# centreborelli/sat-bundleadjust

Hardware: AMD Instinct MI355X
Metric: LM iters/sec at 200 cams x 1M pts x 10M obs (affine, R+T) (higher is better)
Workload: dtype f64; 1 GPU; C4: 200 cams x 1000000 pts x 9998866 obs, affine, correction R+T, 1 fixed camera, seed 1; obs_per_rank0=9998866

## Files before the change

sat-bundleadjust_amd/csrc/satba_capi.hip:

```cpp
#include <hip/hip_runtime.h>

#include <algorithm>
#include <atomic>
#include <chrono>
#include <cmath>
#include <cstdarg>
#include <cstdio>
#include <cstdlib>
#include <cstring>
#include <new>
#include <string>
#include <thread>
#include <vector>

#include "../../include/satba.h"
#include "satba_chol.h"
#include "satba_kernels.h"
#include "satba_layout.h"
#include "satba_lm.h"
#include "satba_lmdev.h"
#include "satba_outliers.h"
#include "satba_triangulate.h"
#include "satba_tracks.h"
#include "satba_ftracks.h"
// ... 399 lines not shown
        while (p->prof_ev.size() < p->prof_used + 2) {
            hipEvent_t e;
            HIP_TRY(hipEventCreate(&e));
            p->prof_ev.push_back(e);
        }
        HIP_TRY(hipEventRecord(p->prof_ev[p->prof_used], p->stream));
    }
    SATBA_DISPATCH(p, TRY((launch_lin<MODEL, NP, CL, RL>(p, a))));
    if (prof) {
        HIP_TRY(hipEventRecord(p->prof_ev[p->prof_used + 1], p->stream));
        p->prof_used += 2;
    }
    return 0;
}

static int launch_cam_sums(satba_problem* p, const int* gate, double* U, double* gc) {
    ObsArgs a = obs_args(p, false, gate);
    CamMajor cm = cam_major(p);
    SATBA_DISPATCH(p, hipLaunchKernelGGL((k_cam_sums<MODEL, NP>), dim3(p->M, p->cm_chunks), dim3(LINC_THREADS), 0, p->stream, a, cm, p->d_f, p->d_part3));
    HIP_TRY(hipGetLastError());
    const int total = p->M * cam_acc_len(p->NP);
    hipLaunchKernelGGL(k_cam_sums_finish, dim3((total + 255) / 256), dim3(256), 0, p->stream, p->M, p->NP, p->cm_chunks, p->d_part3, U, gc, gate);
    HIP_TRY(hipGetLastError());
    return 0;
}

static SchurArgs schur_args(const satba_problem* p) {
    SchurArgs s;
    s.PV = reinterpret_cast<const double2*>(p->d_PV);
    s.pair_ofs = p->L.pair_ofs; s.pair_pts = p->L.pair_pts; s.pair_pi = p->L.pair_pi; s.pair_pj = p->L.pair_pj;
    s.pair_ij = p->L.pair_ij; s.pair_part = p->d_pair_part; s.n_chunks = p->L.C; s.items = p->d_items; s.desc = p->d_item_desc;
    if (wmode(p) && p->L.wl_ready) {
        s.PV = p->d_W; s.wmode = 1; s.zero_fix = p->L.zero_fix; s.n_dg = p->L.n_dg;
        s.pair_rec = p->L.pair_rec; s.pair_kk = p->L.pair_kk; s.cm_rec = p->L.cm_rec; s.cm_sc = p->L.cm_sc; s.dg_part = p->d_part3;
        s.items = p->d_items_w; s.desc = p->d_item_desc_w;
    }
    return s;
}

template <int MODEL, int NP>
static int launch_schur(satba_problem* p, const FrontCtx& f, const ObsArgs& a, double* S, double* rhs) {
    CamMajor cm = cam_major(p);
    SchurArgs s = schur_args(p);
    const long long n_pairs = p->L.n_pairs;
    const bool pairs_run = n_pairs > 0 && p->L.E > 0;
    const bool dg_in_pairs = s.wmode && MODEL != RPC && pairs_run;
    int dchunks = (a.sc && MODEL != RPC) ? p->cm_chunks_w : p->cm_chunks;
    static const bool one_launch_env = !(getenv("SATBA_SCHUR_ONE_LAUNCH") && atoi(getenv("SATBA_SCHUR_ONE_LAUNCH")) == 0);
    const bool both = one_launch_env && !f.arrive_epoch && !dg_in_pairs && pairs_run;
    if (dg_in_pairs) dchunks = p->L.n_dg;
    else {
        if (s.wmode) cm.pt = p->L.cm_rec;
        s.diag_xcd = (dchunks % 8 == 0 && !getenv("SATBA_NO_DIAG_XCD")) ? 1 : 0;
        if (!both) hipLaunchKernelGGL((k_schur_diag<MODEL, NP>), dim3(p->M, dchunks), dim3(LINC_THREADS), 0, p->stream, a, cm, s, p->d_part3);
    }
    const int total = p->M * cam_acc_len(NP);
    const int nb_diag = (int)((std::max<long long>(8ll * total, p->hdr) + 255) / 256);
    auto finish = [&](int red_chunks, bool direct) {
        const long long outs = red_chunks > 1 ? n_pairs * NP * NP : 0;
        const bool scale = f.scale_in_finish && !direct && 1 + CH_MAX_STEPS <= nb_diag * 256;
        hipLaunchKernelGGL(k_schur_finish, dim3((unsigned)(nb_diag + (outs + 255) / 256)), dim3(256), 0, p->stream, p->M, NP, p->n_c, dchunks, p->d_part3,
                           f.lam, f.lam_dev, p->lead, p->d_gc, p->d_scale_inv, S, rhs, p->d_xb, (int)p->hdr, nb_diag, red_chunks,
                           p->L.pair_ij, p->d_pair_part, a.gate, scale ? p->d_dch : (double*)nullptr, scale ? p->d_fail : (int*)nullptr,
                           scale ? 1 + CH_MAX_STEPS : 0);
        p->s_scaled = scale;
    };
    if (f.arrive_epoch) {
        if (dg_in_pairs) {
            const int keep = dchunks;
            dchunks = 0;
            finish(1, true);
            dchunks = keep;
            s.dg_cnt = p->d_dg_cnt; s.dg_lam = f.lam; s.dg_lam_dev = f.lam_dev; s.dg_lead = p->lead; s.dg_gc = p->d_gc;
            s.dg_scale_inv = p->d_scale_inv; s.dg_rhs = rhs;
        } else finish(1, true);
        s.arrive = p->d_arrive; s.arrive_epoch = f.arrive_epoch; s.pair_cnt = p->d_pair_cnt; s.fail = p->d_fail;
    }
    int red_chunks = 1;
    if (n_pairs > 0 && p->L.E > 0) {
        const bool merged = a.unit && p->d_item_desc_merged;
        if (merged) { s.desc = p->d_item_desc_merged; s.items = p->d_items_merged; s.n_chunks = 1; }
        const dim3 igrid((unsigned)(merged ? p->n_item_blocks_merged : (s.wmode ? p->n_item_blocks_w : p->n_item_blocks)));
        if (both) {
            const int n_diag = p->M * dchunks, n_diag_pad = (n_diag + 7) & ~7;
            const dim3 bgrid(igrid.x + (unsigned)n_diag_pad);
            if (a.unit) hipLaunchKernelGGL((k_schur_both<MODEL, NP, true>), bgrid, dim3(256), 0, p->stream, a, cm, s, p->d_part3, S, n_diag, n_diag_pad, p->M, dchunks);
            else hipLaunchKernelGGL((k_schur_both<MODEL, NP, false>), bgrid, dim3(256), 0, p->stream, a, cm, s, p->d_part3, S, n_diag, n_diag_pad, p->M, dchunks);
        }
        else if (a.unit) hipLaunchKernelGGL((k_schur_pairs<MODEL, NP, true>), igrid, dim3(256), 0, p->stream, a, s, S);
        else hipLaunchKernelGGL((k_schur_pairs<MODEL, NP, false>), igrid, dim3(256), 0, p->stream, a, s, S);
        HIP_TRY(hipGetLastError());
        if (p->L.C > 1 && !merged) red_chunks = p->L.C;
        if (f.arrive_epoch && (a.unit ? red_chunks > 1 : false)) return fail(SATBA_E_STATE, "factorisation beside a unit-weight pair kernel with chunk partials");
    }
    if (!f.arrive_epoch) finish(red_chunks, n_pairs > 0 && p->L.E > 0 && red_chunks == 1);
    HIP_TRY(hipGetLastError());
    return 0;
}

static int launch_schur_kernel(satba_problem* p, const int* gate, const FrontCtx& f) {
    ObsArgs a = obs_args(p, false, gate);
    double* S = p->payload();
    double* rhs = S + (size_t)p->n_c * p->n_c;
    SATBA_DISPATCH(p, TRY((launch_schur<MODEL, NP>(p, f, a, S, rhs))));
    return 0;
}

// ... 1407 lines not shown
```

sat-bundleadjust_amd/csrc/satba_schur.h:

```cpp
#pragma once
#include "satba_kernels.h"

namespace satba {

constexpr int PV_STRIDE = 16;
__device__ inline double schur_lambda(const double* __restrict__ hdr, double Delta, double lam_floor, double* __restrict__ keep, bool write) {
    const double gh_sq = hdr[SATBA_HDR_GH_SQ], jg_sq = hdr[SATBA_HDR_JG_SQ], xs_sq = hdr[SATBA_HDR_XS_SQ];
    if (!(Delta > 0.0)) {
        Delta = sqrt(xs_sq);
        if (Delta == 0.0) Delta = 1.0;
    }
    const double a = 0.5 * jg_sq, b = -gh_sq, ub = Delta / sqrt(gh_sq);
    double best = fmin(0.0, a * ub * ub + b * ub);
    if (a != 0.0) {
        const double ext = -0.5 * b / a;
        if (0.0 < ext && ext < ub) best = fmin(best, a * ext * ext + b * ext);
    }
    double lam = -best / (Delta * Delta);
    if (!(lam >= lam_floor)) lam = lam_floor;
    if (write) {
        keep[SATBA_KEEP_GINF] = fmax(keep[SATBA_KEEP_GINF], hdr[SATBA_HDR_GC_INF]);
        keep[SATBA_KEEP_GH_SQ] = gh_sq; keep[SATBA_KEEP_JG_SQ] = jg_sq; keep[SATBA_KEEP_XS_SQ] = xs_sq;
        keep[SATBA_KEEP_LAM] = lam;
        keep[SATBA_KEEP_DELTA] = Delta;
// ... 184 lines not shown
        __hip_atomic_store(cnt, 0, __ATOMIC_RELAXED, __HIP_MEMORY_SCOPE_AGENT);
    }
    __builtin_amdgcn_wave_barrier();
    if (writer) {
        const double* first = mine - (size_t)chunk * stride;
        double t = 0.0;
        for (int ch = 0; ch < n_chunks; ++ch) t += __hip_atomic_load(first + (size_t)ch * stride, __ATOMIC_RELAXED, __HIP_MEMORY_SCOPE_AGENT);
        __hip_atomic_store(s_out, t, __ATOMIC_RELAXED, __HIP_MEMORY_SCOPE_AGENT);
    }
    asm volatile("s_waitcnt vmcnt(0)" ::: "memory");
    if (lane == 0) __hip_atomic_fetch_add(arrive_row, 1, __ATOMIC_RELAXED, __HIP_MEMORY_SCOPE_AGENT);
}

template <bool ATOMIC>
__device__ __forceinline__ double schur_diag_total(const double* __restrict__ part, int cam, int n_chunks, int CU, int k, int sub, bool live) {
    double t = 0.0;
    if (live)
        for (int ch = sub; ch < n_chunks; ch += 8) {
            const double* q = part + ((size_t)cam * n_chunks + ch) * CU + k;
            t += ATOMIC ? __hip_atomic_load(q, __ATOMIC_RELAXED, __HIP_MEMORY_SCOPE_AGENT) : *q;
        }
    t += __shfl_xor(t, 1);
    t += __shfl_xor(t, 2);
    t += __shfl_xor(t, 4);
    return t;
}
template <bool ATOMIC>
__device__ __forceinline__ void schur_diag_store(int cam, int k, double t, int NP, int n_c, double lam, double lead, const double* __restrict__ gc,
                                                 const double* __restrict__ scale_inv, double* __restrict__ S, double* __restrict__ rhs,
                                                 double* __restrict__ rhs_scaled) {
    auto st = [](double* q, double v) { if (ATOMIC) __hip_atomic_store(q, v, __ATOMIC_RELAXED, __HIP_MEMORY_SCOPE_AGENT); else *q = v; };
    const int ntri = NP * (NP + 1) / 2;
    if (k >= ntri) {
        const int col = cam * NP + (k - ntri);
        const double v = lead * gc[col] + t;
        st(rhs + col, v);
        if (rhs_scaled) rhs_scaled[col] = v / scale_inv[col];
        return;
    }
    int r = 0, rem = k;
    while (rem >= NP - r) { rem -= NP - r; ++r; }
    const int q = r + rem;
    double v = 0.0;
    if (q == r) {
        const double si = scale_inv[cam * NP + r];
        v = lead * lam * si * si;
    }
    double out = v + t;
    if (rhs_scaled) out /= scale_inv[cam * NP + q] * scale_inv[cam * NP + r];
    st(S + (size_t)(cam * NP + q) + (size_t)(cam * NP + r) * n_c, out);
    if (q != r) st(S + (size_t)(cam * NP + r) + (size_t)(cam * NP + q) * n_c, out);
}

template <int MODEL, int NP, int THREADS>
__device__ __forceinline__ void schur_diag_walk(const ObsArgs& a, const double2* __restrict__ base, const int* __restrict__ lst_rec,
                                                const int* __restrict__ lst_sc, int rmul, int zero_rec, int cam, int lo, int hi, int tid,
                                                double2* my, double (&acc)[cam_acc_len(NP)]);

#ifndef SATBA_PAIRS_OCC_U
#define SATBA_PAIRS_OCC_U 3
#endif
#ifndef SATBA_PAIRS_OCC_W
#define SATBA_PAIRS_OCC_W 3
#endif
#ifndef SATBA_PAIRS_OCC_MIN_O
#define SATBA_PAIRS_OCC_MIN_O 1
#endif
#define SATBA_PAIRS_WAVES_ATTR(MODEL, NP, UNITW) __attribute__((amdgpu_waves_per_eu(((MODEL) == AFFINE && (NP) <= 6) ? ((UNITW) ? SATBA_PAIRS_OCC_U : SATBA_PAIRS_OCC_W) : SATBA_PAIRS_OCC_MIN_O, ((MODEL) == AFFINE && (NP) <= 6) ? ((UNITW) ? SATBA_PAIRS_OCC_U : SATBA_PAIRS_OCC_W) : 3)))
template <int NP, bool UNITW>
__device__ __forceinline__ void schur_pairs_epilogue_wide(const ObsArgs& a, const SchurArgs& s, double* __restrict__ S, const unsigned bidx, const int lane,
                                                          const int i, const int j, const int chunk, const long long pair, const long long n_pairs,
                                                          const double (&acc)[NP][NP]) {
    constexpr int NB2 = NP * NP, NPS = (NB2 + 63) / 64;
    const double cam_mask = (i < a.n_cam_fix || j < a.n_cam_fix) ? 0.0 : 1.0;
    double total[NPS];
    int ev[NPS];
#pragma unroll
    for (int ps = 0; ps < NPS; ++ps) {
        double flat[64];
#pragma unroll
        for (int e = 0; e < 64; ++e) flat[e] = (64 * ps + e < NB2) ? acc[(64 * ps + e) / NP][(64 * ps + e) % NP] : 0.0;
        total[ps] = cam_mask * wave_reduce_scatter<64>(flat, lane, 32);
        ev[ps] = 64 * ps + rs_index<64>(lane);
    }
    if (s.arrive && bidx == 0 && threadIdx.x == 0)
        __hip_atomic_store(s.arrive + (size_t)SCHUR_ARRIVE_STRIDE * a.M, s.arrive_epoch, __ATOMIC_RELAXED, __HIP_MEMORY_SCOPE_AGENT);
    auto out = [&](int e) { return S + (size_t)(j * NP + e % NP) + (size_t)(i * NP + e / NP) * a.n_c; };
    const size_t stride = (size_t)n_pairs * NB2;
    double* const part = s.pair_part + ((size_t)chunk * n_pairs + pair) * NB2;
    if (!UNITW && s.arrive && s.n_chunks > 1) {
#pragma unroll
        for (int ps = 0; ps < NPS; ++ps)
            if (ev[ps] < NB2) __hip_atomic_store(part + ev[ps], total[ps], __ATOMIC_RELAXED, __HIP_MEMORY_SCOPE_AGENT);
        asm volatile("s_waitcnt vmcnt(0)" ::: "memory");
        int* cnt = s.pair_cnt + pair;
        if (chunk + 1 < s.n_chunks) {
            if (lane == 0) __hip_atomic_fetch_add(cnt, 1, __ATOMIC_RELAXED, __HIP_MEMORY_SCOPE_AGENT);
            return;
        }
        if (lane == 0) {
            int spins = 0;
            while (__hip_atomic_load(cnt, __ATOMIC_RELAXED, __HIP_MEMORY_SCOPE_AGENT) < s.n_chunks - 1) {
                __builtin_amdgcn_s_sleep(4);
                if (++spins > (1 << 22)) { atomicOr(s.fail, SATBA_CHOL_TIMEOUT); break; }
            }
            __hip_atomic_store(cnt, 0, __ATOMIC_RELAXED, __HIP_MEMORY_SCOPE_AGENT);
        }
        __builtin_amdgcn_wave_barrier();
#pragma unroll
        for (int ps = 0; ps < NPS; ++ps) {
            if (ev[ps] >= NB2) continue;
            const double* first = part - (size_t)chunk * stride + ev[ps];
            double t = 0.0;
            for (int ch = 0; ch < s.n_chunks; ++ch) t += __hip_atomic_load(first + (size_t)ch * stride, __ATOMIC_RELAXED, __HIP_MEMORY_SCOPE_AGENT);
            __hip_atomic_store(out(ev[ps]), t, __ATOMIC_RELAXED, __HIP_MEMORY_SCOPE_AGENT);
        }
        asm volatile("s_waitcnt vmcnt(0)" ::: "memory");
        if (lane == 0) __hip_atomic_fetch_add(s.arrive + (size_t)SCHUR_ARRIVE_STRIDE * i, 1, __ATOMIC_RELAXED, __HIP_MEMORY_SCOPE_AGENT);
        return;
    }
#pragma unroll
    for (int ps = 0; ps < NPS; ++ps) {
        if (ev[ps] >= NB2) continue;
        if (s.n_chunks > 1) part[ev[ps]] = total[ps];
        else if (!s.arrive) *out(ev[ps]) = total[ps];
        else __hip_atomic_store(out(ev[ps]), total[ps], __ATOMIC_RELAXED, __HIP_MEMORY_SCOPE_AGENT);
    }
    if (s.arrive && s.n_chunks == 1) {
        asm volatile("s_waitcnt vmcnt(0)" ::: "memory");
        if (lane == 0) __hip_atomic_fetch_add(s.arrive + (size_t)SCHUR_ARRIVE_STRIDE * i, 1, __ATOMIC_RELAXED, __HIP_MEMORY_SCOPE_AGENT);
    }
}

template <int MODEL, int NP, bool UNITW>
__device__ __forceinline__ void schur_pairs_body(const ObsArgs& a, const SchurArgs& s, double* __restrict__ S, const unsigned bidx, double2* s_coop, unsigned (*s_idx)[3 * 64]) {
    const int lane = threadIdx.x & 63, wave = threadIdx.x >> 6;
    const long long n_pairs = (long long)a.M * (a.M - 1) / 2;
    const SchurItem* dp = s.desc + (bidx * 4u + (unsigned)wave);
    const int i = __builtin_amdgcn_readfirstlane(dp->i);
    if (i < 0) return;
    const int j = __builtin_amdgcn_readfirstlane(dp->j);
    const int chunk = __builtin_amdgcn_readfirstlane(dp->chunk);
    const long long pair = __builtin_amdgcn_readfirstlane(dp->pair);
    if constexpr (!UNITW && MODEL != RPC) {
        if (i == j) {
            constexpr int CU = cam_acc_len(NP), CPAD = CU <= 16 ? 16 : 32;
            double dacc[CU];
#pragma unroll
            for (int k = 0; k < CU; ++k) dacc[k] = 0.0;
            schur_diag_walk<MODEL, NP, 64>(a, s.PV, s.cm_rec, s.cm_sc, 1, s.zero_fix, i, (int)dp->lo, (int)dp->hi, lane,
                                           reinterpret_cast<double2*>(reinterpret_cast<char*>(s_coop) + wave * (64 * 112)), dacc);
            const double cam_mask = i < a.n_cam_fix ? 0.0 : 1.0;
            if constexpr (CU > 32) {
#pragma unroll
                for (int o = 0; o < CU; o += 64) {
                    double flat[64];
#pragma unroll
                    for (int e = 0; e < 64; ++e) flat[e] = (o + e < CU) ? dacc[o + e] : 0.0;
                    const double total = cam_mask * wave_reduce_scatter<64>(flat, lane, 32);
                    const int e = o + rs_index<64>(lane);
                    double* const mine = s.dg_part + ((size_t)i * s.n_dg + chunk) * CU + e;
                    if (e < CU) {
                        if (!s.arrive) *mine = total;
                        else __hip_atomic_store(mine, total, __ATOMIC_RELAXED, __HIP_MEMORY_SCOPE_AGENT);
                    }
                }
                if (!s.arrive) return;
            } else {
            double flat[CPAD];
#pragma unroll
            for (int e = 0; e < CPAD; ++e) flat[e] = (e < CU) ? dacc[e] : 0.0;
            const double total = cam_mask * wave_reduce_scatter<CPAD>(flat, lane, 32);
            const int e = rs_index<CPAD>(lane);
            double* const mine = s.dg_part + ((size_t)i * s.n_dg + chunk) * CU + e;
            const bool writer = (lane & (64 / CPAD - 1)) == 0 && e < CU;
            if (!s.arrive) {
                if (writer) *mine = total;
                return;
            }
            if (writer) __hip_atomic_store(mine, total, __ATOMIC_RELAXED, __HIP_MEMORY_SCOPE_AGENT);
            }
            asm volatile("s_waitcnt vmcnt(0)" ::: "memory");
            if (bidx == 0 && threadIdx.x == 0)
                __hip_atomic_store(s.arrive + (size_t)SCHUR_ARRIVE_STRIDE * a.M, s.arrive_epoch, __ATOMIC_RELAXED, __HIP_MEMORY_SCOPE_AGENT);
            int* cnt = s.dg_cnt + i;
            if (chunk + 1 < s.n_dg) {
                if (lane == 0) __hip_atomic_fetch_add(cnt, 1, __ATOMIC_RELAXED, __HIP_MEMORY_SCOPE_AGENT);
                return;
            }
            if (lane == 0) {
                const long long t0 = wall_clock64();
                while (__hip_atomic_load(cnt, __ATOMIC_RELAXED, __HIP_MEMORY_SCOPE_AGENT) < s.n_dg - 1) {
                    __builtin_amdgcn_s_sleep(4);
                    if (wall_clock64() - t0 > 100000000ll) { atomicOr(s.fail, SATBA_CHOL_TIMEOUT); break; }
                }
                __hip_atomic_store(cnt, 0, __ATOMIC_RELAXED, __HIP_MEMORY_SCOPE_AGENT);
            }
            __builtin_amdgcn_wave_barrier();
            const double lam = s.dg_lam_dev ? *s.dg_lam_dev : s.dg_lam;
#pragma unroll 1
            for (int o0 = 0; o0 < CU; o0 += 8) {
                const int k = o0 + (lane >> 3), sub = lane & 7;
                const bool live = k < CU;
                const double t = schur_diag_total<true>(s.dg_part, i, s.n_dg, CU, live ? k : 0, sub, live);
// ... 125 lines not shown
        for (int q = 0; q < NP; ++q) {
            const double y0 = m00 * Jcj[0][q] + m01 * Jcj[1][q];
            const double y1 = m10 * Jcj[0][q] + m11 * Jcj[1][q];
#pragma unroll
            for (int r = 0; r < NP; ++r) acc[r][q] = fma(-Jci[0][r], y0, fma(-Jci[1][r], y1, acc[r][q]));
        }
    };

    {
        const long long lo = dp->lo, hi = dp->hi;
        constexpr bool POS = !UNITW || MODEL == RPC;
        constexpr bool SCL = !UNITW && MODEL != RPC;
        const int n_it = (int)((hi - lo + 63) >> 6);
        if (n_it > 0) {
            const long long last = hi - 1;
            auto ld = [&](const int* arr, long long k) { return __builtin_nontemporal_load(arr + (k < last ? k : last)); };
            auto ldp = [&](long long k) { const int v = ld(SCL ? s.pair_rec : s.pair_pts, k); return (k < hi) ? v : (SCL ? s.zero_fix : a.N); };
            auto ldk = [&](long long k) { const int v = ld(s.pair_kk, k); return (k < hi) ? v : 0x00010001; };
            constexpr int NPC = SCL ? 7 : 5;
            struct Coop { double2 c0, c1, c2, c3, c4, c5, c6; };
            int rsrc[NPC];
            const double2* psrc[NPC];
            unsigned pcv[NPC];
            int kind[NPC];
#pragma unroll
            for (int t = 0; t < NPC; ++t) {
                const int g = 64 * t + lane, pc = g % NPC;
                rsrc[t] = g / NPC;
                pcv[t] = (unsigned)pc;
                kind[t] = 64 * (pc < 5 ? 0 : pc - 4) + g / NPC;
                psrc[t] = pc < 5 ? s.PV + pc : reinterpret_cast<const double2*>(a.sc);
            }
            unsigned* sidx = s_idx[wave];
            auto coop_load = [&](int p, int pi, int pj) {
                Coop o;
                if constexpr (SCL) {
                    asm volatile("" ::: "memory");
                    sidx[lane] = (unsigned)p; sidx[64 + lane] = (unsigned)p - ((unsigned)pi & 0xffffu); sidx[128 + lane] = (unsigned)p - ((unsigned)pi >> 16);
                    asm volatile("" ::: "memory");
                    __builtin_amdgcn_wave_barrier();
                    const unsigned o0 = sidx[kind[0]], o1 = sidx[kind[1]], o2 = sidx[kind[2]], o3 = sidx[kind[3]], o4 = sidx[kind[4]],
                                   o5 = sidx[kind[NPC - 2]], o6 = sidx[kind[NPC - 1]];
                    asm volatile("" ::: "memory");
                    __builtin_amdgcn_wave_barrier();
                    o.c0 = psrc[0][o0]; o.c1 = psrc[1][o1]; o.c2 = psrc[2][o2]; o.c3 = psrc[3][o3]; o.c4 = psrc[4][o4];
                    o.c5 = psrc[NPC - 2][o5]; o.c6 = psrc[NPC - 1][o6];
                } else {
#define SATBA_CL(t) s.PV[(unsigned)(PV_STRIDE / 2) * (unsigned)__shfl(p, rsrc[t]) + pcv[t]]
                    o.c0 = SATBA_CL(0); o.c1 = SATBA_CL(1); o.c2 = SATBA_CL(2); o.c3 = SATBA_CL(3); o.c4 = SATBA_CL(4);
#undef SATBA_CL
                }
                return o;
            };
            char* my = reinterpret_cast<char*>(s_coop) + wave * (64 * 112);
            double2* wr = reinterpret_cast<double2*>(my) + lane;
            const double2* mine = reinterpret_cast<const double2*>(my + lane * (16 * NPC));
            double2 si_cur = make_double2(1.0, 1.0), sj_cur = si_cur;
            auto transpose = [&](const Coop& o) {
                Rec r;
                asm volatile("" ::: "memory");
                wr[0] = o.c0; wr[64] = o.c1; wr[128] = o.c2; wr[192] = o.c3; wr[256] = o.c4;
                if constexpr (SCL) { wr[320] = o.c5; wr[384] = o.c6; }
                asm volatile("" ::: "memory");
                __builtin_amdgcn_wave_barrier();
                r.r0 = mine[0]; r.r1 = mine[1]; r.r2 = mine[2]; r.r3 = mine[3]; r.r4 = mine[4].x;
                if constexpr (SCL) { si_cur = mine[5]; sj_cur = mine[6]; }
                asm volatile("" ::: "memory");
                __builtin_amdgcn_wave_barrier();
                return r;
            };
            struct JCoop { double2 c0, c1, c2; };
            struct JRow { double v[JLEN]; };
            int jsrc[3];
            const double2* jp[3];
            double2* jw[3];
#pragma unroll
            for (int t = 0; t < 3; ++t) {
                const int g = 64 * t + lane;
                jsrc[t] = g / 3; jp[t] = reinterpret_cast<const double2*>(a.Jpm) + g % 3; jw[t] = reinterpret_cast<double2*>(my) + g;
            }
            auto jcoop_load = [&](int io) {
                JCoop o;
                constexpr size_t RS = jrow_stride(NP) / 2;
                o.c0 = jp[0][RS * (size_t)__shfl(io, jsrc[0])];
                o.c1 = jp[1][RS * (size_t)__shfl(io, jsrc[1])];
                o.c2 = jp[2][RS * (size_t)__shfl(io, jsrc[2])];
                return o;
            };
            const double2* jmine = reinterpret_cast<const double2*>(my) + lane * 3;
            auto jtranspose = [&](const JCoop& o) {
                JRow r;
                asm volatile("" ::: "memory");
                *jw[0] = o.c0; *jw[1] = o.c1; *jw[2] = o.c2;
                asm volatile("" ::: "memory");
                __builtin_amdgcn_wave_barrier();
#pragma unroll
                for (int k = 0; k < 3; ++k) { const double2 t = jmine[k]; r.v[2 * k] = t.x; r.v[2 * k + 1] = t.y; }
                asm volatile("" ::: "memory");
                __builtin_amdgcn_wave_barrier();
                return r;
            };
            long long idx = lo + lane;
            int p_nxt = ldp(idx + 64);
            int pi_cur = 0, pj_cur = 0, pi_nxt = 0, pj_nxt = 0;
            if constexpr (SCL) {
                pi_cur = ldk(idx); pi_nxt = ldk(idx + 64);
            } else if constexpr (POS) {
                pi_cur = ld(s.pair_pi, idx); pj_cur = ld(s.pair_pj, idx);
                pi_nxt = ld(s.pair_pi, idx + 64); pj_nxt = ld(s.pair_pj, idx + 64);
            }
            Coop c_cur = coop_load(ldp(idx), pi_cur, pj_cur);
            JCoop ji_cur, jj_cur;
            if constexpr (JROWS) { ji_cur = jcoop_load(pi_cur); jj_cur = jcoop_load(pj_cur); }
            for (int it = 0; it < n_it; ++it) {
                const Rec r_cur = transpose(c_cur);
                JRow ti, tj;
                if constexpr (JROWS) { ti = jtranspose(ji_cur); tj = jtranspose(jj_cur); }
                const int p_nn = ldp(idx + 128);
                int pi_nn = 0, pj_nn = 0;
                if constexpr (SCL) pi_nn = ldk(idx + 128);
                else if constexpr (POS) { pi_nn = ld(s.pair_pi, idx + 128); pj_nn = ld(s.pair_pj, idx + 128); }
                const Coop c_nxt = coop_load(p_nxt, pi_nxt, pj_nxt);
                JCoop ji_nxt, jj_nxt;
                if constexpr (JROWS) { ji_nxt = jcoop_load(pi_nxt); jj_nxt = jcoop_load(pj_nxt); }
                __builtin_amdgcn_sched_barrier(0);
                compute(r_cur, pi_cur, pj_cur, si_cur, sj_cur, ti.v, tj.v);
                __builtin_amdgcn_sched_barrier(0);
                p_nxt = p_nn; c_cur = c_nxt;
                if constexpr (JROWS) { ji_cur = ji_nxt; jj_cur = jj_nxt; }
                pi_cur = pi_nxt; pj_cur = pj_nxt; pi_nxt = pi_nn; pj_nxt = pj_nn;
                idx += 64;
            }
        }
    }

    constexpr int NB2 = NP * NP;
    if constexpr (NB2 > 64) {
        schur_pairs_epilogue_wide<NP, UNITW>(a, s, S, bidx, lane, i, j, chunk, pair, n_pairs, acc);
        return;
    }
    constexpr int NPAD = NB2 <= 16 ? 16 : (NB2 <= 32 ? 32 : 64);
    static_assert(NB2 <= NPAD || NB2 > 64, "pair block reduction");
    double flat[NPAD];
#pragma unroll
    for (int e = 0; e < NPAD; ++e) flat[e] = (e < NB2) ? acc[e / NP][e % NP] : 0.0;
    const double cam_mask = (i < a.n_cam_fix || j < a.n_cam_fix) ? 0.0 : 1.0;
    const double total = cam_mask * wave_reduce_scatter<NPAD>(flat, lane, 32);
    const int e = rs_index<NPAD>(lane);
    const bool writer = (lane & (64 / NPAD - 1)) == 0 && e < NB2;
    int e_ = e, i_ = i, j_ = j, chunk_ = chunk;
    long long pair_ = pair;
    asm volatile("" : "+v"(e_), "+s"(i_), "+s"(j_), "+s"(chunk_), "+s"(pair_));
    if (s.arrive && bidx == 0 && threadIdx.x == 0)
        __hip_atomic_store(s.arrive + (size_t)SCHUR_ARRIVE_STRIDE * a.M, s.arrive_epoch, __ATOMIC_RELAXED, __HIP_MEMORY_SCOPE_AGENT);
    double* const s_out = S + (size_t)(j_ * NP + e_ % NP) + (size_t)(i_ * NP + e_ / NP) * a.n_c;
    if constexpr (!UNITW) {
        if (s.arrive && s.n_chunks > 1) {
            schur_pair_publish(s.pair_part + ((size_t)chunk_ * n_pairs + pair_) * NB2 + e_, (size_t)n_pairs * NB2, s.n_chunks, chunk_, s.pair_cnt + pair_,
                               s.arrive + (size_t)SCHUR_ARRIVE_STRIDE * i_, s.fail, s_out, total, writer);
            return;
        }
    }
    if (writer) {
        if (s.n_chunks > 1) s.pair_part[((size_t)chunk_ * n_pairs + pair_) * NB2 + e_] = total;
        else if (!s.arrive) *s_out = total;
        else __hip_atomic_store(s_out, total, __ATOMIC_RELAXED, __HIP_MEMORY_SCOPE_AGENT);
    }
    if (s.arrive && s.n_chunks == 1) {
        asm volatile("s_waitcnt vmcnt(0)" ::: "memory");
        if (lane == 0) __hip_atomic_fetch_add(s.arrive + (size_t)SCHUR_ARRIVE_STRIDE * i_, 1, __ATOMIC_RELAXED, __HIP_MEMORY_SCOPE_AGENT);
    }
}
template <int MODEL, int NP, bool UNITW>
__global__ __launch_bounds__(256) SATBA_PAIRS_WAVES_ATTR(MODEL, NP, UNITW) void k_schur_pairs(ObsArgs a, SchurArgs s, double* __restrict__ S) {
    SATBA_GATE(a.gate);
    __shared__ double2 s_coop[4 * 64 * 7];
    __shared__ unsigned s_idx[4][3 * 64];
    schur_pairs_body<MODEL, NP, UNITW>(a, s, S, blockIdx.x, s_coop, s_idx);
}


template <int MODEL, int NP, int THREADS>
__device__ __forceinline__ void schur_diag_walk(const ObsArgs& a, const double2* __restrict__ base, const int* __restrict__ lst_rec,
                                                const int* __restrict__ lst_sc, int rmul, int zero_rec, int cam, int lo, int hi, int tid,
                                                double2* my, double (&acc)[cam_acc_len(NP)]) {
    const double* cc = a.camc + (size_t)cam * CAMC;
    struct Rec { double2 r0, r1, r2, r3, r4, r5; };
    const int lane = tid & 63;
    int rsrc[6];
    const double2* psrc[6];
    double2* wdst[6];
#pragma unroll
    for (int t = 0; t < 6; ++t) {
        const int g = 64 * t + lane;
        rsrc[t] = g / 6; psrc[t] = base + g % 6; wdst[t] = my + (g / 6) * 7 + g % 6;
    }
    struct Coop { double2 c0, c1, c2, c3, c4, c5; };
    auto coop_load = [&](int p) {
        Coop o;
        o.c0 = psrc[0][(size_t)__shfl(p, rsrc[0])];
        o.c1 = psrc[1][(size_t)__shfl(p, rsrc[1])];
        o.c2 = psrc[2][(size_t)__shfl(p, rsrc[2])];
        o.c3 = psrc[3][(size_t)__shfl(p, rsrc[3])];
        o.c4 = psrc[4][(size_t)__shfl(p, rsrc[4])];
        o.c5 = psrc[5][(size_t)__shfl(p, rsrc[5])];
        return o;
    };
    const double2* mine = my + lane * 7;
    auto transpose = [&](const Coop& o) {
        Rec r;
        asm volatile("" ::: "memory");
        *wdst[0] = o.c0; *wdst[1] = o.c1; *wdst[2] = o.c2; *wdst[3] = o.c3; *wdst[4] = o.c4; *wdst[5] = o.c5;
        asm volatile("" ::: "memory");
        __builtin_amdgcn_wave_barrier();
        r.r0 = mine[0]; r.r1 = mine[1]; r.r2 = mine[2]; r.r3 = mine[3]; r.r4 = mine[4]; r.r5 = mine[5];
        asm volatile("" ::: "memory");
        __builtin_amdgcn_wave_barrier();
        return r;
    };
    constexpr bool AFAC = MODEL == AFFINE && NP <= 5;
    double Pm[2][3], Au[3] = {0.0, 0.0, 0.0}, tr[6] = {0.0, 0.0, 0.0, 0.0, 0.0, 0.0};
    if constexpr (AFAC) {
        const double fx = cc[CAMX + 2], fy = cc[CAMX + 3], sk = cc[CAMX + 4];
        Au[0] = fx; Au[1] = sk; Au[2] = fy;
#pragma unroll
        for (int k = 0; k < 3; ++k) { Pm[0][k] = fx * cc[6 + k] + sk * cc[9 + k]; Pm[1][k] = fy * cc[9 + k]; }
#pragma unroll
        for (int k = 0; k < 6; ++k) tr[k] = cc[k];
    }
    const int n_it = (hi - lo + THREADS - 1) / THREADS;
    if (n_it > 0) {
        auto ldp = [&](int q) { const int v = lst_rec[q < hi ? q : hi - 1]; return q < hi ? rmul * v : zero_rec; };
        int pos = lo + tid;
        int p_nxt = ldp(pos + THREADS);
        Coop cur = coop_load(ldp(pos));
        const bool scl = MODEL != RPC && a.sc != nullptr;
        auto ldio = [&](int q) { return lst_sc[q < hi ? q : hi - 1]; };
        int io_nxt = scl ? ldio(pos + THREADS) : 0;
        double2 sc_cur = scl ? a.sc[ldio(pos)] : make_double2(1.0, 1.0);
        for (int it = 0; it < n_it; ++it, pos += THREADS) {
            const Rec rc = transpose(cur);
            const int p_nn = ldp(pos + 2 * THREADS);
            const int io_nn = scl ? ldio(pos + 2 * THREADS) : 0;
            const double2 sc_nxt = scl ? a.sc[io_nxt] : make_double2(1.0, 1.0);
            const Coop nxt = coop_load(p_nxt);
            __builtin_amdgcn_sched_barrier(0);
            const double2 sc_now = sc_cur;
            sc_cur = sc_nxt; io_nxt = io_nn;
            const double2 r0 = rc.r0, r1 = rc.r1, r2 = rc.r2, r3 = rc.r3, r4 = rc.r4, r5 = rc.r5;
            p_nxt = p_nn; cur = nxt;
            const bool valid = pos < hi;
            const int posc = valid ? pos : hi - 1;
            const double vm = valid ? 1.0 : 0.0;
            double sx = vm, sy = vm;
            double ux = vm, uy = vm;
            const double v00 = r1.y, v01 = r2.x, v02 = r2.y, v11 = r3.x, v12 = r3.y, v22 = r4.x;
            if constexpr (AFAC) {
                if (a.sc) { const double2 t = sc_now; ux = vm * t.x * t.x; uy = vm * t.y * t.y; }
                sx = ux; sy = uy;
                double T[2][3];
#pragma unroll
                for (int r = 0; r < 2; ++r) {
                    T[r][0] = Pm[r][0] * v00 + Pm[r][1] * v01 + Pm[r][2] * v02;
                    T[r][1] = Pm[r][0] * v01 + Pm[r][1] * v11 + Pm[r][2] * v12;
                    T[r][2] = Pm[r][0] * v02 + Pm[r][1] * v12 + Pm[r][2] * v22;
                }
                const double n00 = ux - sx * ux * (T[0][0] * Pm[0][0] + T[0][1] * Pm[0][1] + T[0][2] * Pm[0][2]);
                const double n01 = -sx * uy * (T[0][0] * Pm[1][0] + T[0][1] * Pm[1][1] + T[0][2] * Pm[1][2]);
                const double n11 = uy - sy * uy * (T[1][0] * Pm[1][0] + T[1][1] * Pm[1][1] + T[1][2] * Pm[1][2]);
                const double ag0 = sx * (T[0][0] * r4.y + T[0][1] * r5.x + T[0][2] * r5.y);
                const double ag1 = sy * (T[1][0] * r4.y + T[1][1] * r5.x + T[1][2] * r5.y);
                const double t00 = Au[0] * n00, t01 = Au[0] * n01;
                const double t10 = Au[1] * n00 + Au[2] * n01, t11 = Au[1] * n01 + Au[2] * n11;
                const double e00 = t00 * Au[0], e01 = t00 * Au[1] + t01 * Au[2], e11 = t10 * Au[1] + t11 * Au[2];
                const double b0 = Au[0] * ag0, b1 = Au[1] * ag0 + Au[2] * ag1;
                double D[2][3];
                {
                    const double X = r0.x, Y = r0.y, Z = r1.x;
                    const double ca = tr[0], sa = tr[1], cb = tr[2], sb = tr[3], cg = tr[4], sg = tr[5];
                    const double y1y = ca * Y - sa * Z, y1z = sa * Y + ca * Z;
                    const double y2x = cb * X + sb * y1z, y2z = -sb * X + cb * y1z;
                    const double ax = sb * y1y;
                    D[0][0] = cg * ax + sg * y1z; D[1][0] = sg * ax - cg * y1z;
                    D[0][1] = cg * y2z;           D[1][1] = sg * y2z;
                    D[0][2] = -(sg * y2x + cg * y1y); D[1][2] = cg * y2x - sg * y1y;
                }
                double y0[3], y1[3];
#pragma unroll
                for (int q = 0; q < 3; ++q) { y0[q] = e00 * D[0][q] + e01 * D[1][q]; y1[q] = e01 * D[0][q] + e11 * D[1][q]; }
                int k = 0;
#pragma unroll
                for (int r = 0; r < 3; ++r) {
#pragma unroll
                    for (int q = r; q < 3; ++q) acc[k++] += D[0][r] * y0[q] + D[1][r] * y1[q];
                    if constexpr (NP == 5) { acc[k++] += y0[r]; acc[k++] += y1[r]; }
                }
                if constexpr (NP == 5) { acc[k++] += e00; acc[k++] += e01; acc[k++] += e11; }
#pragma unroll
                for (int r = 0; r < 3; ++r) acc[k++] -= D[0][r] * b0 + D[1][r] * b1;
                if constexpr (NP == 5) { acc[k++] -= b0; acc[k++] -= b1; }
            } else {
                double Jc[2][NP], Jp[2][3];
                if constexpr (MODEL == RPC) {
                    ObsEval<MODEL, NP, true> e2;
                    e2.load_d(a, lst_sc[posc]);
                    rpc_jac_from_d<NP>(cc, r0.x, r0.y, r1.x, e2.Dr, Jc, Jp);
#pragma unroll
                    for (int k = 0; k < NP; ++k) { Jc[0][k] *= vm; Jc[1][k] *= vm; }
                    ux = uy = sx = sy = 1.0;
                } else {
                    double u, v;
                    project<MODEL, NP, true>(cc, nullptr, r0.x, r0.y, r1.x, false, u, v, Jc, Jp);
                    if (a.sc) { const double2 t = sc_now; ux = vm * t.x * t.x; uy = vm * t.y * t.y; }
                    sx = ux; sy = uy;
                }
                double A[2][3];
#pragma unroll
                for (int r = 0; r < 2; ++r) {
                    A[r][0] = Jp[r][0] * v00 + Jp[r][1] * v01 + Jp[r][2] * v02;
                    A[r][1] = Jp[r][0] * v01 + Jp[r][1] * v11 + Jp[r][2] * v12;
                    A[r][2] = Jp[r][0] * v02 + Jp[r][1] * v12 + Jp[r][2] * v22;
                }
                const double m00 = sx * ux * (A[0][0] * Jp[0][0] + A[0][1] * Jp[0][1] + A[0][2] * Jp[0][2]);
                const double m01 = sx * uy * (A[0][0] * Jp[1][0] + A[0][1] * Jp[1][1] + A[0][2] * Jp[1][2]);
                const double m11 = sy * uy * (A[1][0] * Jp[1][0] + A[1][1] * Jp[1][1] + A[1][2] * Jp[1][2]);
                const double ag0 = sx * (A[0][0] * r4.y + A[0][1] * r5.x + A[0][2] * r5.y);
                const double ag1 = sy * (A[1][0] * r4.y + A[1][1] * r5.x + A[1][2] * r5.y);
                int k = 0;
#pragma unroll
                for (int r = 0; r < NP; ++r) {
                    const double y0 = m00 * Jc[0][r] + m01 * Jc[1][r];
                    const double y1 = m01 * Jc[0][r] + m11 * Jc[1][r];
#pragma unroll
                    for (int q = r; q < NP; ++q) {
                        acc[k] -= Jc[0][q] * y0 + Jc[1][q] * y1;
                        acc[k] += ux * Jc[0][r] * Jc[0][q] + uy * Jc[1][r] * Jc[1][q];
                        ++k;
                    }
                }
#pragma unroll
                for (int r = 0; r < NP; ++r) acc[k++] -= Jc[0][r] * ag0 + Jc[1][r] * ag1;
            }
            __builtin_amdgcn_sched_barrier(0);
        }
    }
}

template <int MODEL, int NP>
__device__ __forceinline__ void schur_diag_body(const ObsArgs& a, const CamMajor& c, const SchurArgs& s, double* __restrict__ part, const int L, const int M,
                                                const int n_chunks, double2* s_coop, double (*s_red)[cam_acc_len(NP)]) {
    constexpr int CU = cam_acc_len(NP);
    int cam = L % M, chunk = L / M;
    if (s.diag_xcd) {
        const int x = L & 7, q = L >> 3;
        cam = q % M; chunk = (q / M) * 8 + x;
    }
    const int b = c.cam_ofs[cam], e = c.cam_ofs[cam + 1];
    const long long len = e - b;
    const int lo = b + (int)(len * chunk / n_chunks), hi = b + (int)(len * (chunk + 1) / n_chunks);
    const int lane = threadIdx.x & 63, wave = threadIdx.x >> 6;
    double acc[CU];
#pragma unroll
    for (int k = 0; k < CU; ++k) acc[k] = 0.0;
    schur_diag_walk<MODEL, NP, LINC_THREADS>(a, s.PV, c.pt, c.io, s.wmode ? 1 : PV_STRIDE / 2, s.wmode ? s.zero_fix : (PV_STRIDE / 2) * a.N, cam, lo, hi,
                                             (int)threadIdx.x, s_coop + wave * (64 * 7), acc);
    if (cam < a.n_cam_fix) {
#pragma unroll
        for (int k = 0; k < CU; ++k) acc[k] = 0.0;
    }
#pragma unroll
    for (int k = 0; k < CU; ++k) {
        const double t = wave_sum(acc[k]);
        if (lane == 0) s_red[wave][k] = t;
    }
    __syncthreads();
    if (threadIdx.x < CU) {
        double t = 0.0;
        for (int wv = 0; wv < LINC_THREADS / 64; ++wv) t += s_red[wv][threadIdx.x];
        part[((size_t)cam * n_chunks + chunk) * CU + threadIdx.x] = t;
    }
}
template <int MODEL, int NP>
__global__ __launch_bounds__(LINC_THREADS) void k_schur_diag(ObsArgs a, CamMajor c, SchurArgs s, double* __restrict__ part) {
    SATBA_GATE(a.gate);
    __shared__ double2 s_coop[(LINC_THREADS / 64) * 64 * 7];
    __shared__ double s_red[LINC_THREADS / 64][cam_acc_len(NP)];
    schur_diag_body<MODEL, NP>(a, c, s, part, (int)(blockIdx.y * gridDim.x + blockIdx.x), (int)gridDim.x, (int)gridDim.y, s_coop, s_red);
}
static_assert(LINC_THREADS == 256, "k_schur_both: both bodies run 256 threads");
template <int MODEL, int NP, bool UNITW>
__global__ __launch_bounds__(256) SATBA_PAIRS_WAVES_ATTR(MODEL, NP, UNITW) void k_schur_both(ObsArgs a, CamMajor c, SchurArgs s, double* __restrict__ part, double* __restrict__ S,
                                                                                      int n_diag, int n_diag_pad, int M, int n_chunks) {
    SATBA_GATE(a.gate);
    __shared__ double2 s_coop[4 * 64 * 7];
    __shared__ unsigned s_idx[4][3 * 64];
    __shared__ double s_red[4][cam_acc_len(NP)];
    if ((int)blockIdx.x < n_diag_pad) {
        if ((int)blockIdx.x < n_diag) schur_diag_body<MODEL, NP>(a, c, s, part, (int)blockIdx.x, M, n_chunks, s_coop, s_red);
        return;
    }
    schur_pairs_body<MODEL, NP, UNITW>(a, s, S, blockIdx.x - (unsigned)n_diag_pad, s_coop, s_idx);
}

__global__ __launch_bounds__(256) void k_schur_finish(int M, int NP, int n_c, int n_chunks, const double* __restrict__ part, double lam,
                                                      const double* __restrict__ lam_dev, double lead, const double* __restrict__ gc,
                                                      const double* __restrict__ scale_inv, double* __restrict__ S, double* __restrict__ rhs,
                                                      double* __restrict__ xb, int hdr_len, int nb_diag, int red_chunks,
                                                      const int2* __restrict__ pair_ij, const double* __restrict__ pair_part, const int* gate,
                                                      double* __restrict__ rhs_scaled = nullptr, int* __restrict__ clear = nullptr, int n_clear = 0) {
    SATBA_GATE(gate);
    if ((int)blockIdx.x >= nb_diag) {
        const long long n_pairs = (long long)M * (M - 1) / 2;
        const int NB2 = NP * NP;
        const long long idx = (long long)(blockIdx.x - nb_diag) * blockDim.x + threadIdx.x;
        if (idx >= n_pairs * NB2) return;
        const long long pair = idx / NB2;
        const int e = (int)(idx % NB2);
        double t = 0.0;
        int ch = 0;
        for (; ch + 4 <= red_chunks; ch += 4) {
            const double p0 = pair_part[((size_t)ch * n_pairs + pair) * NB2 + e], p1 = pair_part[((size_t)(ch + 1) * n_pairs + pair) * NB2 + e];
            const double p2 = pair_part[((size_t)(ch + 2) * n_pairs + pair) * NB2 + e], p3 = pair_part[((size_t)(ch + 3) * n_pairs + pair) * NB2 + e];
            t += p0; t += p1; t += p2; t += p3;
        }
        for (; ch < red_chunks; ++ch) t += pair_part[((size_t)ch * n_pairs + pair) * NB2 + e];
        const int2 ij = pair_ij[pair];
        const int r = e / NP, q = e % NP;
        if (rhs_scaled) t /= scale_inv[ij.y * NP + q] * scale_inv[ij.x * NP + r];
        S[(size_t)(ij.y * NP + q) + (size_t)(ij.x * NP + r) * n_c] = t;
        return;
    }
    if (lam_dev) lam = *lam_dev;
    const int CU = cam_acc_len(NP);
    const int gid = blockIdx.x * blockDim.x + threadIdx.x, idx = gid >> 3, sub = gid & 7;
    if (gid < hdr_len) xb[gid] = 0.0;
    if (gid < n_clear) clear[gid] = 0;
    if (n_chunks <= 0) return;
    const bool live = idx < M * CU;
    const int cam = live ? idx / CU : 0, k = live ? idx % CU : 0;
    const double t = schur_diag_total<false>(part, cam, n_chunks, CU, k, sub, live);
    if (!live || sub != 0) return;
    schur_diag_store<false>(cam, k, t, NP, n_c, lam, lead, gc, scale_inv, S, rhs, rhs_scaled);
}

}
```

Baseline: 912.8 LM iters/sec.

## Stage Schur point records into LDS via global_load_lds DMA for affine unit weights

Adds a path in the Schur diagonal walk and the pair accumulation where gathered point records are copied straight from global memory into LDS with global_load_lds. This replaces register cooperative loads and transposes. It targets affine models with NP<=6 and unit weights, and is enabled by default through SATBA_SCHUR_LDSDMA=3. The aim is to cut VGPR pressure and shuffle or transpose work in the gather-heavy Schur build. In exchange it relies on hand-placed s_waitcnt sequencing, with a risk of serialising load latency (vmcnt(0) waits each iteration) and of subtle ordering bugs.

```diff
diff --git a/sat-bundleadjust_amd/csrc/satba_capi.hip b/sat-bundleadjust_amd/csrc/satba_capi.hip
--- a/sat-bundleadjust_amd/csrc/satba_capi.hip
+++ b/sat-bundleadjust_amd/csrc/satba_capi.hip
@@ -475,7 +475,9 @@
     else {
         if (s.wmode) cm.pt = p->L.cm_rec;
         s.diag_xcd = (dchunks % 8 == 0 && !getenv("SATBA_NO_DIAG_XCD")) ? 1 : 0;
-        if (!both) hipLaunchKernelGGL((k_schur_diag<MODEL, NP>), dim3(p->M, dchunks), dim3(LINC_THREADS), 0, p->stream, a, cm, s, p->d_part3);
+        if (both) {}
+        else if (schur_lds_dma_diag(MODEL, NP, true) && a.unit) hipLaunchKernelGGL((k_schur_diag<MODEL, NP, schur_lds_dma_diag(MODEL, NP, true)>), dim3(p->M, dchunks), dim3(LINC_THREADS), 0, p->stream, a, cm, s, p->d_part3);
+        else hipLaunchKernelGGL((k_schur_diag<MODEL, NP>), dim3(p->M, dchunks), dim3(LINC_THREADS), 0, p->stream, a, cm, s, p->d_part3);
     }
     const int total = p->M * cam_acc_len(NP);
     const int nb_diag = (int)((std::max<long long>(8ll * total, p->hdr) + 255) / 256);
diff --git a/sat-bundleadjust_amd/csrc/satba_schur.h b/sat-bundleadjust_amd/csrc/satba_schur.h
--- a/sat-bundleadjust_amd/csrc/satba_schur.h
+++ b/sat-bundleadjust_amd/csrc/satba_schur.h
@@ -260,7 +260,7 @@
     if (q != r) st(S + (size_t)(cam * NP + r) + (size_t)(cam * NP + q) * n_c, out);
 }
 
-template <int MODEL, int NP, int THREADS>
+template <int MODEL, int NP, int THREADS, bool DMA = false>
 __device__ __forceinline__ void schur_diag_walk(const ObsArgs& a, const double2* __restrict__ base, const int* __restrict__ lst_rec,
                                                 const int* __restrict__ lst_sc, int rmul, int zero_rec, int cam, int lo, int hi, int tid,
                                                 double2* my, double (&acc)[cam_acc_len(NP)]);
@@ -275,6 +275,19 @@
 #define SATBA_PAIRS_OCC_MIN_O 1
 #endif
 #define SATBA_PAIRS_WAVES_ATTR(MODEL, NP, UNITW) __attribute__((amdgpu_waves_per_eu(((MODEL) == AFFINE && (NP) <= 6) ? ((UNITW) ? SATBA_PAIRS_OCC_U : SATBA_PAIRS_OCC_W) : SATBA_PAIRS_OCC_MIN_O, ((MODEL) == AFFINE && (NP) <= 6) ? ((UNITW) ? SATBA_PAIRS_OCC_U : SATBA_PAIRS_OCC_W) : 3)))
+#ifndef SATBA_SCHUR_LDSDMA
+#define SATBA_SCHUR_LDSDMA 3
+#endif
+constexpr bool schur_lds_dma_diag(int model, int np, bool unitw) { return (SATBA_SCHUR_LDSDMA & 1) && unitw && model == AFFINE && np <= 6; }
+constexpr bool schur_lds_dma(int model, int np, bool unitw) { return (SATBA_SCHUR_LDSDMA & 2) && unitw && model == AFFINE && np <= 6; }
+#ifndef SATBA_PAIRS_LDS_STAGES
+#define SATBA_PAIRS_LDS_STAGES 1
+#endif
+static_assert(SATBA_PAIRS_LDS_STAGES == 1 || SATBA_PAIRS_LDS_STAGES == 2, "one LDS image or a ring of two");
+constexpr int schur_coop_pieces(int model, int np, bool unitw) { return (schur_lds_dma(model, np, unitw) && SATBA_PAIRS_LDS_STAGES == 2) ? 64 * 11 : 64 * 7; }
+__device__ __forceinline__ void schur_glds16(const double2* src, double2* dst) {
+    __builtin_amdgcn_global_load_lds((const __attribute__((address_space(1))) void*)src, (__attribute__((address_space(3))) void*)dst, 16, 0, 0);
+}
 template <int NP, bool UNITW>
 __device__ __forceinline__ void schur_pairs_epilogue_wide(const ObsArgs& a, const SchurArgs& s, double* __restrict__ S, const unsigned bidx, const int lane,
                                                           const int i, const int j, const int chunk, const long long pair, const long long n_pairs,
@@ -357,7 +370,7 @@
 #pragma unroll
             for (int k = 0; k < CU; ++k) dacc[k] = 0.0;
             schur_diag_walk<MODEL, NP, 64>(a, s.PV, s.cm_rec, s.cm_sc, 1, s.zero_fix, i, (int)dp->lo, (int)dp->hi, lane,
-                                           reinterpret_cast<double2*>(reinterpret_cast<char*>(s_coop) + wave * (64 * 112)), dacc);
+                                           s_coop + wave * schur_coop_pieces(MODEL, NP, UNITW), dacc);
             const double cam_mask = i < a.n_cam_fix ? 0.0 : 1.0;
             if constexpr (CU > 32) {
 #pragma unroll
@@ -589,7 +602,7 @@
                 }
                 return o;
             };
-            char* my = reinterpret_cast<char*>(s_coop) + wave * (64 * 112);
+            char* my = reinterpret_cast<char*>(s_coop + wave * schur_coop_pieces(MODEL, NP, UNITW));
             double2* wr = reinterpret_cast<double2*>(my) + lane;
             const double2* mine = reinterpret_cast<const double2*>(my + lane * (16 * NPC));
             double2 si_cur = make_double2(1.0, 1.0), sj_cur = si_cur;
@@ -638,6 +651,64 @@
                 return r;
             };
             long long idx = lo + lane;
+            if constexpr (schur_lds_dma(MODEL, NP, UNITW)) {
+                double2* const dst = reinterpret_cast<double2*>(my);
+                auto dma = [&](int p, double2* to) {
+#pragma unroll
+                    for (int t = 0; t < NPC; ++t)
+                        schur_glds16(s.PV + ((unsigned)(PV_STRIDE / 2) * (unsigned)__shfl(p, rsrc[t]) + pcv[t]), to + 64 * t);
+                };
+                if constexpr (SATBA_PAIRS_LDS_STAGES == 2) {
+                    static_assert(NPC == 5, "vmcnt(6) below");
+                    unsigned* const ring = reinterpret_cast<unsigned*>(dst + 2 * 64 * NPC);
+                    auto idx_dma = [&](long long k, int slot) {
+                        __builtin_amdgcn_global_load_lds((const __attribute__((address_space(1))) void*)(s.pair_pts + (k < last ? k : last)),
+                                                         (__attribute__((address_space(3))) void*)(ring + 64 * slot), 4, 0, 2);
+                    };
+                    auto idx_get = [&](long long k, int slot) { const int v = (int)ring[64 * slot + lane]; return k < hi ? v : a.N; };
+                    idx_dma(idx, 0); idx_dma(idx + 64, 1); idx_dma(idx + 128, 2);
+                    asm volatile("s_waitcnt vmcnt(0)" ::: "memory");
+                    const int p_0 = idx_get(idx, 0), p_1 = idx_get(idx + 64, 1);
+                    dma(p_0, dst);
+                    asm volatile("" ::: "memory");
+                    idx_dma(idx + 192, 3);
+                    asm volatile("" ::: "memory");
+                    dma(p_1, dst + 64 * NPC);
+                    for (int it = 0; it < n_it; ++it) {
+                        Rec r_cur;
+                        const int st = (it & 1) * (64 * NPC);
+                        asm volatile("s_waitcnt vmcnt(6)" ::: "memory");
+                        r_cur.r0 = mine[st]; r_cur.r1 = mine[st + 1]; r_cur.r2 = mine[st + 2]; r_cur.r3 = mine[st + 3]; r_cur.r4 = mine[st + 4].x;
+                        const int p_2 = idx_get(idx + 128, (it + 2) & 3);
+                        asm volatile("s_waitcnt lgkmcnt(0)" ::: "memory");
+                        idx_dma(idx + 256, it & 3);
+                        asm volatile("" ::: "memory");
+                        dma(p_2, dst + st);
+                        asm volatile("" ::: "memory");
+                        __builtin_amdgcn_sched_barrier(0);
+                        compute(r_cur, 0, 0, si_cur, sj_cur, nullptr, nullptr);
+                        __builtin_amdgcn_sched_barrier(0);
+                        idx += 64;
+                    }
+                    asm volatile("s_waitcnt vmcnt(0)" ::: "memory");
+                } else {
+                int p_nx = ldp(idx + 64);
+                dma(ldp(idx), dst);
+                for (int it = 0; it < n_it; ++it) {
+                    Rec r_cur;
+                    asm volatile("s_waitcnt vmcnt(0)" ::: "memory");
+                    r_cur.r0 = mine[0]; r_cur.r1 = mine[1]; r_cur.r2 = mine[2]; r_cur.r3 = mine[3]; r_cur.r4 = mine[4].x;
+                    asm volatile("s_waitcnt lgkmcnt(0)" ::: "memory");
+                    const int p_nn = ldp(idx + 128);
+                    if (it + 1 < n_it) dma(p_nx, dst);
+                    __builtin_amdgcn_sched_barrier(0);
+                    compute(r_cur, 0, 0, si_cur, sj_cur, nullptr, nullptr);
+                    __builtin_amdgcn_sched_barrier(0);
+                    p_nx = p_nn;
+                    idx += 64;
+                }
+                }
+            } else {
             int p_nxt = ldp(idx + 64);
             int pi_cur = 0, pj_cur = 0, pi_nxt = 0, pj_nxt = 0;
             if constexpr (SCL) {
@@ -668,6 +739,7 @@
                 pi_cur = pi_nxt; pj_cur = pj_nxt; pi_nxt = pi_nn; pj_nxt = pj_nn;
                 idx += 64;
             }
+            }
         }
     }
 
@@ -711,13 +783,13 @@
 template <int MODEL, int NP, bool UNITW>
 __global__ __launch_bounds__(256) SATBA_PAIRS_WAVES_ATTR(MODEL, NP, UNITW) void k_schur_pairs(ObsArgs a, SchurArgs s, double* __restrict__ S) {
     SATBA_GATE(a.gate);
-    __shared__ double2 s_coop[4 * 64 * 7];
+    __shared__ double2 s_coop[4 * schur_coop_pieces(MODEL, NP, UNITW)];
     __shared__ unsigned s_idx[4][3 * 64];
     schur_pairs_body<MODEL, NP, UNITW>(a, s, S, blockIdx.x, s_coop, s_idx);
 }
 
 
-template <int MODEL, int NP, int THREADS>
+template <int MODEL, int NP, int THREADS, bool DMA>
 __device__ __forceinline__ void schur_diag_walk(const ObsArgs& a, const double2* __restrict__ base, const int* __restrict__ lst_rec,
                                                 const int* __restrict__ lst_sc, int rmul, int zero_rec, int cam, int lo, int hi, int tid,
                                                 double2* my, double (&acc)[cam_acc_len(NP)]) {
@@ -742,6 +814,18 @@
         o.c4 = psrc[4][(size_t)__shfl(p, rsrc[4])];
         o.c5 = psrc[5][(size_t)__shfl(p, rsrc[5])];
         return o;
+    };
+    int dsrc[7];
+    unsigned dpc[7];
+#pragma unroll
+    for (int t = 0; t < 7; ++t) {
+        const int g = 64 * t + lane;
+        dsrc[t] = g / 7; dpc[t] = (unsigned)(g % 7);
+    }
+    static_assert(!DMA || PV_STRIDE == 16, "the seventh piece is the record's own pad");
+    auto dma = [&](int p) {
+#pragma unroll
+        for (int t = 0; t < 7; ++t) schur_glds16(base + ((unsigned)__shfl(p, dsrc[t]) + dpc[t]), my + 64 * t);
     };
     const double2* mine = my + lane * 7;
     auto transpose = [&](const Coop& o) {
@@ -770,22 +854,32 @@
         auto ldp = [&](int q) { const int v = lst_rec[q < hi ? q : hi - 1]; return q < hi ? rmul * v : zero_rec; };
         int pos = lo + tid;
         int p_nxt = ldp(pos + THREADS);
-        Coop cur = coop_load(ldp(pos));
-        const bool scl = MODEL != RPC && a.sc != nullptr;
+        Coop cur;
+        if constexpr (DMA) dma(ldp(pos));
+        else cur = coop_load(ldp(pos));
+        const bool scl = !DMA && MODEL != RPC && a.sc != nullptr;
         auto ldio = [&](int q) { return lst_sc[q < hi ? q : hi - 1]; };
         int io_nxt = scl ? ldio(pos + THREADS) : 0;
         double2 sc_cur = scl ? a.sc[ldio(pos)] : make_double2(1.0, 1.0);
         for (int it = 0; it < n_it; ++it, pos += THREADS) {
-            const Rec rc = transpose(cur);
+            Rec rc;
+            if constexpr (DMA) {
+                asm volatile("s_waitcnt vmcnt(0)" ::: "memory");
+                rc.r0 = mine[0]; rc.r1 = mine[1]; rc.r2 = mine[2]; rc.r3 = mine[3]; rc.r4 = mine[4]; rc.r5 = mine[5];
+                asm volatile("s_waitcnt lgkmcnt(0)" ::: "memory");
+            } else rc = transpose(cur);
             const int p_nn = ldp(pos + 2 * THREADS);
             const int io_nn = scl ? ldio(pos + 2 * THREADS) : 0;
             const double2 sc_nxt = scl ? a.sc[io_nxt] : make_double2(1.0, 1.0);
-            const Coop nxt = coop_load(p_nxt);
+            Coop nxt;
+            if constexpr (DMA) { if (it + 1 < n_it) dma(p_nxt); }
+            else nxt = coop_load(p_nxt);
             __builtin_amdgcn_sched_barrier(0);
             const double2 sc_now = sc_cur;
             sc_cur = sc_nxt; io_nxt = io_nn;
             const double2 r0 = rc.r0, r1 = rc.r1, r2 = rc.r2, r3 = rc.r3, r4 = rc.r4, r5 = rc.r5;
-            p_nxt = p_nn; cur = nxt;
+            p_nxt = p_nn;
+            if constexpr (!DMA) cur = nxt;
             const bool valid = pos < hi;
             const int posc = valid ? pos : hi - 1;
             const double vm = valid ? 1.0 : 0.0;
@@ -883,7 +977,7 @@
     }
 }
 
-template <int MODEL, int NP>
+template <int MODEL, int NP, bool DMA = false>
 __device__ __forceinline__ void schur_diag_body(const ObsArgs& a, const CamMajor& c, const SchurArgs& s, double* __restrict__ part, const int L, const int M,
                                                 const int n_chunks, double2* s_coop, double (*s_red)[cam_acc_len(NP)]) {
     constexpr int CU = cam_acc_len(NP);
@@ -899,7 +993,7 @@
     double acc[CU];
 #pragma unroll
     for (int k = 0; k < CU; ++k) acc[k] = 0.0;
-    schur_diag_walk<MODEL, NP, LINC_THREADS>(a, s.PV, c.pt, c.io, s.wmode ? 1 : PV_STRIDE / 2, s.wmode ? s.zero_fix : (PV_STRIDE / 2) * a.N, cam, lo, hi,
+    schur_diag_walk<MODEL, NP, LINC_THREADS, DMA>(a, s.PV, c.pt, c.io, s.wmode ? 1 : PV_STRIDE / 2, s.wmode ? s.zero_fix : (PV_STRIDE / 2) * a.N, cam, lo, hi,
                                              (int)threadIdx.x, s_coop + wave * (64 * 7), acc);
     if (cam < a.n_cam_fix) {
 #pragma unroll
@@ -917,23 +1011,23 @@
         part[((size_t)cam * n_chunks + chunk) * CU + threadIdx.x] = t;
     }
 }
-template <int MODEL, int NP>
+template <int MODEL, int NP, bool DMA = false>
 __global__ __launch_bounds__(LINC_THREADS) void k_schur_diag(ObsArgs a, CamMajor c, SchurArgs s, double* __restrict__ part) {
     SATBA_GATE(a.gate);
     __shared__ double2 s_coop[(LINC_THREADS / 64) * 64 * 7];
     __shared__ double s_red[LINC_THREADS / 64][cam_acc_len(NP)];
-    schur_diag_body<MODEL, NP>(a, c, s, part, (int)(blockIdx.y * gridDim.x + blockIdx.x), (int)gridDim.x, (int)gridDim.y, s_coop, s_red);
+    schur_diag_body<MODEL, NP, DMA>(a, c, s, part, (int)(blockIdx.y * gridDim.x + blockIdx.x), (int)gridDim.x, (int)gridDim.y, s_coop, s_red);
 }
 static_assert(LINC_THREADS == 256, "k_schur_both: both bodies run 256 threads");
 template <int MODEL, int NP, bool UNITW>
 __global__ __launch_bounds__(256) SATBA_PAIRS_WAVES_ATTR(MODEL, NP, UNITW) void k_schur_both(ObsArgs a, CamMajor c, SchurArgs s, double* __restrict__ part, double* __restrict__ S,
                                                                                       int n_diag, int n_diag_pad, int M, int n_chunks) {
     SATBA_GATE(a.gate);
-    __shared__ double2 s_coop[4 * 64 * 7];
+    __shared__ double2 s_coop[4 * schur_coop_pieces(MODEL, NP, UNITW)];
     __shared__ unsigned s_idx[4][3 * 64];
     __shared__ double s_red[4][cam_acc_len(NP)];
     if ((int)blockIdx.x < n_diag_pad) {
-        if ((int)blockIdx.x < n_diag) schur_diag_body<MODEL, NP>(a, c, s, part, (int)blockIdx.x, M, n_chunks, s_coop, s_red);
+        if ((int)blockIdx.x < n_diag) schur_diag_body<MODEL, NP, schur_lds_dma_diag(MODEL, NP, UNITW)>(a, c, s, part, (int)blockIdx.x, M, n_chunks, s_coop, s_red);
         return;
     }
     schur_pairs_body<MODEL, NP, UNITW>(a, s, S, blockIdx.x - (unsigned)n_diag_pad, s_coop, s_idx);
```

Result: no change. 917.8 LM iters/sec, median of 6 (+0.6%).
